# mklawonn/Scene-Graph-GAN

Hardware: AMD Instinct MI355X
Metric: triples/sec (G+D step) (higher is better)
Workload: dtype f32 (conv operands scaled per tensor and split into 2 fp16 pieces, round-to-nearest = 23 significant bits, 3 fp16 MFMAs per product, f32 accumulate; native-f32 figure and parity in the same line); 1 GPU; BASELINE.json configs[1] (1xMI355X, batch 64, 224x224, vocab 1000): batch 64 per GPU, 224x224 synthetic images, vocab 1000, 3-token triples, 1 critic update + 1 generator update per step (WGAN-GP lambda=10, TF-Adam); global_batch=64, critic_iters=1, parallelism=dp1, conv_precision_mode=2, schedule=two-stream; per-kernel figures from serial steps

## Files before the change

### scene-graph-gan_amd/build.py

```python
from __future__ import annotations

import hashlib
import os
import subprocess
import sys
from concurrent.futures import ThreadPoolExecutor

HERE = os.path.dirname(os.path.abspath(__file__))
CSRC = os.path.join(HERE, "csrc")
OUT_DIR = os.path.join(HERE, "_build")
LIB_PATH = os.path.join(HERE, "libsgg_hip.so")
ARCH = "gfx950"
HIPCC = os.environ.get("HIPCC", "/opt/rocm/bin/hipcc")
NO_PACKED_FP32 = ["-Xclang", "-target-feature", "-Xclang", "-packed-fp32-ops"]
FLAGS = ["-O3", "-std=c++17", "-fPIC", "--offload-arch=" + ARCH, "-fno-gpu-rdc", "-Wall", "-Wno-unused-function",
         "-ffp-contract=fast"] + NO_PACKED_FP32


def sources():
    return sorted(os.path.join(CSRC, f) for f in os.listdir(CSRC) if f.endswith(".hip"))


def _digest(paths):
    h = hashlib.sha256()
    for p in sorted(paths):
        with open(p, "rb") as f:
            h.update(p.encode())
            h.update(f.read())
    h.update(" ".join(FLAGS).encode())
    return h.hexdigest()


def _compile(src):
    obj = os.path.join(OUT_DIR, os.path.basename(src) + ".o")
    cmd = [HIPCC] + FLAGS + ["-I", CSRC, "-c", src, "-o", obj]
    r = subprocess.run(cmd, capture_output=True, text=True)
    if r.returncode != 0:
        raise RuntimeError("hipcc failed for %s:\n%s\n%s" % (src, r.stdout, r.stderr))
    err = "\n".join(l for l in r.stderr.splitlines() if "is not a recognized feature for this target" not in l)
    return obj, err


OBJDUMP = os.environ.get("LLVM_OBJDUMP", os.path.join(os.path.dirname(os.path.dirname(os.path.realpath(HIPCC))), "lib", "llvm", "bin",
                                                      "llvm-objdump"))


M0_ASM_KERNELS = ("conv_wgrad_dma", "conv_s2_kernel")


def check_device_code(lib_path: str = LIB_PATH) -> int:
    import re
    import shutil
    tmp = os.path.join(OUT_DIR, "disasm")
    shutil.rmtree(tmp, ignore_errors=True)
    os.makedirs(tmp)
    copy = os.path.join(tmp, "lib.so")
    shutil.copy(lib_path, copy)
    if not os.path.exists(OBJDUMP):
# ... 54 lines not shown
    srcs = sources()
    headers = [os.path.join(CSRC, f) for f in os.listdir(CSRC) if f.endswith(".h")]
    stamp = os.path.join(OUT_DIR, "stamp")
    dig = _digest(srcs + headers)
    if not force and os.path.exists(LIB_PATH) and os.path.exists(stamp) and open(stamp).read() == dig:
        return LIB_PATH
    with ThreadPoolExecutor(max_workers=min(6, len(srcs))) as ex:
        results = list(ex.map(_compile, srcs))
    if verbose:
        for _, err in results:
            if err.strip():
                print(err, file=sys.stderr)
    objs = [o for o, _ in results]
    cmd = [HIPCC, "-shared", "-fPIC", "--offload-arch=" + ARCH, "-o", LIB_PATH] + objs
    r = subprocess.run(cmd, capture_output=True, text=True)
    if r.returncode != 0:
        raise RuntimeError("link failed:\n%s\n%s" % (r.stdout, r.stderr))
    check_device_code(LIB_PATH)
    with open(stamp, "w") as f:
        f.write(dig)
    return LIB_PATH


if __name__ == "__main__":
    print(build(force="--force" in sys.argv, verbose=True))
```

### scene-graph-gan_amd/csrc/conv_gather.hip

```cpp
#include "split16.h"
#include "mma_f32.h"
#include "conv_halo.h"
#include <stdlib.h>

struct GatherClass {
  int Hm, Wm, M;
  int nth, ntw;
  int oy, ox;
  int kh0, kw0, kstep;
  int ooy, oox;
  int mtiles;
};

struct GatherParams {
  const float* src;
  const float* wm;
  const float* bias;
  float* out;
  const void* w_split;
  const float* amax_src;
  const float* amax_w;
  int B, Hs, Ws, C;
  int N;
  int Ho, Wo;
// ... 800 lines not shown
    h.src_s16 = operand_format & 1;
    h.cu_cap = cu_cap;
    SGG_CHECK_ARG((size_t)B * Hi * Wi * Cin * sizeof(float) < 0x80000000ull, "sgg_conv2d_nhwc_fwd: input exceeds 2 GiB");
    sgg_halo_launch(h, precision, st);
    SGG_LAUNCH_CHECK("sgg_conv2d_nhwc_fwd(halo)");
    return SGG_OK;
  }
  if (w_split_layout == 3) {
    SGG_CHECK_ARG(w_split && sgg_s2d_applicable(KH, KW, stride, Hi, Wi, Cin, Cout, precision) && pad_t == 1 && pad_l == 1,
                  "sgg_conv2d_nhwc_fwd: w_split_layout 3 needs 5x5 stride 2, 32 -> 32 channels, H %% 16 == W %% 16 == 0, precision 2 or 3 "
                  "(sgg_conv_wsplit_layout)");
    SGG_CHECK_ARG((size_t)B * Hi * Wi * Cin * sizeof(float) < 0x80000000ull, "sgg_conv2d_nhwc_fwd: input exceeds 2 GiB");
    HaloParams h;
    h.src = x; h.wfrag = w_split; h.bias = bias; h.out = y; h.amax_src = amax_x; h.amax_w = amax_w; h.tile_stats = tile_stats;
    h.ln_stats = ln_stats; h.ln_gamma = ln_gamma; h.ln_beta = ln_beta;
    h.B = B; h.H = Ho; h.W = Wo; h.C = 4 * Cin; h.N = Cout; h.bh = Ho / 8; h.bw = Wo / 8; h.nblk = B * h.bh * h.bw; h.flip = 0;
    h.src_bytes = (unsigned)((size_t)B * Hi * Wi * Cin * sizeof(float));
    h.w_bytes = (unsigned)((size_t)9 * 4 * Cin * Cout * sizeof(float));
    sgg_halo_dense_strides(h);
    h.in_rs = 2 * Wi * Cin; h.in_ps = 2 * Cin; h.in_cA = Wi * Cin; h.in_cB = Cin;
    h.ln_nc = Cin;
    h.src_s16 = operand_format & 1;
    h.cu_cap = cu_cap;
    sgg_halo_launch(h, precision, st);
    SGG_LAUNCH_CHECK("sgg_conv2d_nhwc_fwd(s2d)");
    return SGG_OK;
  }
  if (w_split_layout == 2) {
    SGG_CHECK_ARG(w_split && sgg_s2_applicable(KH, KW, stride, B, Hi, Wi, Cin, Cout, precision) && pad_t == 1 && pad_l == 1,
                  "sgg_conv2d_nhwc_fwd: w_split_layout 2 needs 5x5 stride 2 on an even grid, Cout %% 128 == 0, precision 2 or 3 "
                  "(sgg_conv_wsplit_layout)");
    SGG_CHECK_ARG((size_t)B * Hi * Wi * Cin * sizeof(float) < 0x80000000ull && (size_t)B * Ho * Wo * Cout * sizeof(float) < 0x80000000ull,
                  "sgg_conv2d_nhwc_fwd: tensor exceeds 2 GiB");
    SGG_CHECK_ARG(!tile_stats || sgg_s2_stats_per_sample(Ho, Wo, Cout) > 0, "sgg_conv2d_nhwc_fwd: tile_stats need Ho*Wo %% 224 == 0 here");
    S2Params q;
    q.src = x; q.wfrag = w_split; q.bias = bias; q.out = y; q.amax_src = amax_x; q.amax_w = amax_w; q.tile_stats = tile_stats;
    q.ln_stats = ln_stats; q.ln_gamma = ln_gamma; q.ln_beta = ln_beta;
    q.B = B; q.Ho = Ho; q.Wo = Wo; q.C = Cin; q.N = Cout; q.M = B * Ho * Wo; q.nbands = sgg_cdiv(q.M, 224); q.pitch = Wo;
    q.src_bytes = (unsigned)((size_t)B * Hi * Wi * Cin * sizeof(float));
    q.w_bytes = (unsigned)((size_t)25 * Cin * Cout * sizeof(float));
    q.src_s16 = operand_format & 1;
    q.cu_cap = cu_cap;
    sgg_s2_launch(q, 0, precision, st);
    SGG_LAUNCH_CHECK("sgg_conv2d_nhwc_fwd(s2)");
    return SGG_OK;
  }
// ... 46 lines not shown
    h.src_bytes = (unsigned)((size_t)B * Ho * Wo * Cout * sizeof(float));
    h.w_bytes = (unsigned)((size_t)9 * Cin * Cout * sizeof(float));
    sgg_halo_dense_strides(h);
    h.frag16 = w_split_layout == 4;
    h.src_s16 = operand_format & 1;
    sgg_halo_launch(h, precision, (hipStream_t)stream);
    SGG_LAUNCH_CHECK("sgg_conv2d_nhwc_dgrad(halo)");
    return SGG_OK;
  }
  if (w_split_layout == 3) {
    SGG_CHECK_ARG(w_split && sgg_s2d_applicable(KH, KW, stride, Hi, Wi, Cin, Cout, precision) && pad_t == 1 && pad_l == 1 &&
                      Hi == 2 * Ho && Wi == 2 * Wo,
                  "sgg_conv2d_nhwc_dgrad: w_split_layout 3 needs 5x5 stride 2, 32 -> 32 channels, H %% 16 == W %% 16 == 0, precision 2 or 3 "
                  "(sgg_conv_wsplit_layout)");
    HaloParams h;
    h.src = dy; h.wfrag = w_split; h.bias = nullptr; h.out = dx; h.amax_src = amax_dy; h.amax_w = amax_w; h.tile_stats = nullptr;
    h.ln_stats = nullptr; h.ln_gamma = nullptr; h.ln_beta = nullptr;
    h.B = B; h.H = Ho; h.W = Wo; h.C = Cout; h.N = 4 * Cin; h.bh = Ho / 8; h.bw = Wo / 8; h.nblk = B * h.bh * h.bw; h.flip = 1;
    h.src_bytes = (unsigned)((size_t)B * Ho * Wo * Cout * sizeof(float));
    h.w_bytes = (unsigned)((size_t)9 * 4 * Cin * Cout * sizeof(float));
    sgg_halo_dense_strides(h);
    h.out_rs = 2 * Wi * Cin; h.out_ps = 2 * Cin; h.out_nA = Wi * Cin; h.out_nB = Cin;
    h.src_s16 = operand_format & 1;
    sgg_halo_launch(h, precision, (hipStream_t)stream);
    SGG_LAUNCH_CHECK("sgg_conv2d_nhwc_dgrad(s2d)");
    return SGG_OK;
  }
  if (w_split_layout == 2) {
    SGG_CHECK_ARG(w_split && sgg_s2_applicable(KH, KW, stride, B, Hi, Wi, Cout, Cin, precision) && pad_t == 1 && pad_l == 1 &&
                      Hi == 2 * Ho && Wi == 2 * Wo,
                  "sgg_conv2d_nhwc_dgrad: w_split_layout 2 needs 5x5 stride 2 on an even grid, Cin %% 128 == 0, precision 2 or 3 "
                  "(sgg_conv_wsplit_layout)");
    SGG_CHECK_ARG((size_t)B * Hi * Wi * Cin * sizeof(float) < 0x80000000ull && (size_t)B * Ho * Wo * Cout * sizeof(float) < 0x80000000ull,
                  "sgg_conv2d_nhwc_dgrad: tensor exceeds 2 GiB");
    S2Params q;
    q.src = dy; q.wfrag = w_split; q.bias = nullptr; q.out = dx; q.amax_src = amax_dy; q.amax_w = amax_w; q.tile_stats = nullptr;
    q.ln_stats = nullptr; q.ln_gamma = nullptr; q.ln_beta = nullptr;
    q.B = B; q.Ho = Ho; q.Wo = Wo; q.C = Cout; q.N = Cin; q.M = B * Ho * Wo; q.nbands = sgg_cdiv(q.M, 224); q.pitch = Wo;
    q.src_bytes = (unsigned)((size_t)B * Ho * Wo * Cout * sizeof(float));
    q.w_bytes = (unsigned)((size_t)25 * Cin * Cout * sizeof(float));
    q.src_s16 = operand_format & 1;
    q.cu_cap = 0;
    sgg_s2_launch(q, 1, precision, (hipStream_t)stream);
    SGG_LAUNCH_CHECK("sgg_conv2d_nhwc_dgrad(s2)");
    return SGG_OK;
  }
// ... 27 lines not shown
```

### scene-graph-gan_amd/csrc/conv_halo.h

```cpp
#pragma once
#include "sgg_common.h"

struct HaloParams {
  const float* src;
  const void* wfrag;
  const float* bias;
  float* out;
  const float* amax_src;
  const float* amax_w;
  float* tile_stats;
  const float* ln_stats;
  const float* ln_gamma;
  const float* ln_beta;
  int B, H, W, C, N;
  int bh, bw, nblk;
  int flip;
  unsigned src_bytes, w_bytes;
  int gx;
  int in_rs, in_ps, in_cA, in_cB;
  int out_rs, out_ps, out_nA, out_nB;
  int ln_nc;
  int frag16;
  int src_s16;
  int cu_cap;
};
inline int sgg_persist_cus(int cu_cap) { return (cu_cap > 0 && cu_cap < SGG_PERSIST_CUS_PER_XCD) ? cu_cap : SGG_PERSIST_CUS_PER_XCD; }
inline void sgg_halo_dense_strides(HaloParams& h) {
  h.in_rs = h.W * h.C; h.in_ps = h.C; h.in_cA = 64; h.in_cB = 32;
  h.out_rs = h.W * h.N; h.out_ps = h.N; h.out_nA = 64; h.out_nB = 32;
  h.ln_nc = h.C;
  h.frag16 = 0;
  h.src_s16 = 0;
  h.cu_cap = 0;
}

int sgg_halo_applicable(int KH, int KW, int stride, int H, int W, int C, int N, int precision);
int sgg_s2d_applicable(int KH, int KW, int stride, int Hi, int Wi, int Cin, int Cout, int precision);
int sgg_halo_stats_cols(int N);
void sgg_halo_launch(const HaloParams& p, int precision, hipStream_t st);
int sgg_halo_pc_applicable(int C, int N, int precision);
int sgg_halo_pc64_applicable(int C, int N, int precision);
void sgg_halo_pc_launch(const HaloParams& p, int precision, hipStream_t st);

struct WgradHaloPlan {
  int ct, nt;
  int nbs;
  int spw;
  int pairs, pairs_n;
  int nsplit;
  int stages;
  int nslabs;
  int geo;
  int R, pc, xslots;
  size_t ws_bytes;
};
int sgg_wgrad_halo_plan(int B, int H, int W, int Cin, int Cout, int KH, int KW, int stride, WgradHaloPlan* pl);
// ... 43 lines not shown
```

### scene-graph-gan_amd/csrc/conv_halo.hip

```cpp
#include "split16.h"
#include "conv_halo.h"
#include <type_traits>
#include <stdlib.h>

constexpr int SGG_HALO_DB_MAX = 65536;
#define HALO_PITCH 12
#define HALO_BLKB (10 * HALO_PITCH * 64)

__device__ __forceinline__ int halo_sw(int ry, int rx) { return ((rx >> 2) & 1) | ((ry & 1) << 1); }

template <int NB, int BN, int WGM, int WGN, bool HALF, bool PREFETCH, bool ONECH, bool LNP, bool ONE = false, int WB = 1>
__global__ __launch_bounds__(64 * WGM * WGN, 2) void conv_halo3_kernel(HaloParams p) {
  static_assert(PREFETCH && WB == 1, "patch prefetch, one block per wave");
  constexpr int P = ONE ? 1 : 2;
  constexpr int WN = BN / WGN, TM = 2 * WB, TN = WN / 32;
  constexpr int THREADS = 64 * WGM * WGN;
  static_assert((WGM * WGN == 4 || WGM * WGN == 2) && NB * 64 / WGM == 64 * WB && WN % 32 == 0 && TN >= 1,
                "a wave owns WB 8x8 blocks x WN columns");
  constexpr int PLANEB = NB * HALO_BLKB;
  constexpr int ITEMS = NB * 400;
  constexpr int NPASS = (ITEMS + THREADS - 1) / THREADS;
  constexpr bool DB = (2 * P * PLANEB <= SGG_HALO_DB_MAX) && THREADS == 256;
  __shared__ __attribute__((aligned(16))) unsigned char lds[(DB ? 2 : 1) * P * PLANEB];
  __shared__ __attribute__((aligned(16))) float lnp_s[LNP ? 1024 : 4];

  const int ntiles_n = p.N / BN;
  const int mtiles = (p.nblk + NB - 1) / NB;
  const int xcd = blockIdx.x & 7, jx = blockIdx.x >> 3;
  const int nt = jx % ntiles_n;
  const int tstride = p.gx / ntiles_n;
  const int mt_begin = (int)(((long long)xcd * mtiles) >> 3) + jx / ntiles_n;
  const int mt_end = (int)(((long long)(xcd + 1) * mtiles) >> 3);
  if (mt_begin >= mt_end) return;
  const int n0 = nt * BN;
  const int tid = threadIdx.x, lane = tid & 63;
  const int wave = __builtin_amdgcn_readfirstlane(tid >> 6);
// ... 27 lines not shown
      lnp_s[512 + c] = p.ln_beta[c];
    }
    __syncthreads();
  }
  float ld_mu[NB], ld_rs[NB];
  int ld_cc = 0, ld_bad = 0;

  int s_grow[NB], s_by[NB], s_bx[NB];
#pragma unroll
  for (int j = 0; j < NB; ++j) {
    const int beta = mt_begin * NB + j;
    s_grow[j] = beta / p.bw;
    s_bx[j] = beta % p.bw;
    s_by[j] = s_grow[j] % p.bh;
  }
  int s_tile = mt_begin, s_cc = 0;
  const int nch = p.C >> 5;
  const int adv_rows = (tstride * NB) / p.bw, adv_cols = (tstride * NB) % p.bw;

  f32x4 pre[NPASS][2];
  auto stage_load = [&]() __attribute__((always_inline)) {
    unsigned base[NB];
    int bbits[NB];
#pragma unroll
    for (int j = 0; j < NB; ++j) {
      const bool dead = (s_tile >= mt_end) | (s_tile * NB + j >= p.nblk);
      base[j] = (unsigned)(((s_grow[j] * 8 - 1) * p.in_rs + (s_bx[j] * 8 - 1) * p.in_ps + (s_cc >> 1) * p.in_cA + (s_cc & 1) * p.in_cB) * 4);
      bbits[j] = dead ? 15 : ((s_by[j] == 0) | ((s_by[j] == p.bh - 1) << 1) | ((s_bx[j] == 0) << 2) | ((s_bx[j] == p.bw - 1) << 3));
      if (dead) base[j] = SGG_OOB;
    }
    if constexpr (LNP) {
      ld_cc = s_cc;
      ld_bad = 0;
#pragma unroll
      for (int j = 0; j < NB; ++j) {
        int b = s_grow[j] / p.bh;
        b = b < p.B ? b : p.B - 1;
        ld_mu[j] = p.ln_stats[2 * b];
        ld_rs[j] = p.ln_stats[2 * b + 1];
      }
    }
#pragma unroll
    for (int j = 0; j < NPASS; ++j) {
      const int blk = (it_meta[j] >> 24) & 3;
      unsigned b0 = base[0];
      int bb = bbits[0];
#pragma unroll
      for (int k = 1; k < NB; ++k) {
        b0 = blk == k ? base[k] : b0;
        bb = blk == k ? bbits[k] : bb;
// ... 29 lines not shown
        const int blk = (it_meta[j] >> 24) & 3;
        float mu = ld_mu[0], rs = ld_rs[0];
#pragma unroll
        for (int k = 1; k < NB; ++k) {
          mu = blk == k ? ld_mu[k] : mu;
          rs = blk == k ? ld_rs[k] : rs;
        }
        const int cb = ((ld_cc * 32) & (p.ln_nc - 1)) + ((it_meta[j] >> 26) & 3) * 8;
        ln_elu8(pre[j][0], pre[j][1], lnp_s + cb, lnp_s + 512 + cb, mu, rs, (ld_bad >> j) & 1);
      }
      u32x4 pl[P];
      if constexpr (LNP || !HALF) split8<P, HALF>(pre[j][0], pre[j][1], sa, pl);
      else stage_planes<P, HALF>(pre[j][0], pre[j][1], sa, p.src_s16, pl);
      if ((it_meta[j] >> 28) & 1) {
#pragma unroll
        for (int pp = 0; pp < P; ++pp) *reinterpret_cast<u32x4*>(dst + pp * PLANEB + (it_meta[j] & 0xfffff)) = pl[pp];
      }
    }
  };

  const unsigned w_lane = (unsigned)((n0 + wn0) >> 5) * 4096u + (unsigned)lane * 16u;
  const unsigned w_slab = (unsigned)(p.N >> 5) * 4096u;
  u32x4 rb[2][TN][2][P];
  auto load_b = [&](auto par_c, int cc, int tap) {
    constexpr int par = decltype(par_c)::value;
    const unsigned base = (unsigned)(tap * nch + cc) * w_slab + w_lane;
#pragma unroll
    for (int tn = 0; tn < TN; ++tn)
#pragma unroll
      for (int ks = 0; ks < 2; ++ks)
#pragma unroll
        for (int pp = 0; pp < P; ++pp)
          rb[par][tn][ks][pp] = __builtin_bit_cast(u32x4, buf_load4(rs_w, base + (unsigned)(tn * 4096 + ks * 2048 + pp * 1024)));
  };

  f32x16 acc[TM][TN];
  acc_zero<TM, TN>(acc);

  const int i = lane & 31, h = lane >> 5;
  const int pyl = i >> 3, pxl = i & 7;
  int cur = 0;

  u32x4 a[2][TM][2][P];
  auto read_a_ks = [&](auto buf_c, int tap, auto ks0_c, auto nks_c) {
    constexpr int buf = decltype(buf_c)::value, ks0 = decltype(ks0_c)::value, nks = decltype(nks_c)::value;
    const int kh = tap / 3, kw = tap % 3;
    const int dyy = p.flip ? 2 - kh : kh, dxx = p.flip ? 2 - kw : kw;
    int pyv = pyl, pxv = pxl;
    asm volatile("" : "+v"(pyv), "+v"(pxv));
    const unsigned char* patch_w = lds + (DB ? cur * (P * PLANEB) : 0) + wblk * HALO_BLKB;
#pragma unroll
    for (int tm = 0; tm < TM; ++tm) {
      const int ry = (tm & 1) * 4 + pyv + dyy, rx = pxv + dxx;
      const unsigned char* row = patch_w + (tm >> 1) * HALO_BLKB + (ry * HALO_PITCH + rx) * 64;
      const int hs = halo_sw(ry, rx);
#pragma unroll
      for (int ks = ks0; ks < ks0 + nks; ++ks)
#pragma unroll
        for (int pp = 0; pp < P; ++pp)
          a[buf][tm][ks][pp] = *reinterpret_cast<const u32x4*>(row + pp * PLANEB + (((2 * ks + h) ^ hs) << 4));
    }
  };
  auto read_a = [&](auto buf_c, int tap) { read_a_ks(buf_c, tap, std::integral_constant<int, 0>{}, std::integral_constant<int, 2>{}); };
  auto mma_kstep = [&](auto par_c, auto ks_c) {
    constexpr int par = decltype(par_c)::value, ks = decltype(ks_c)::value;
#pragma unroll
    for (int tm = 0; tm < TM; ++tm)
#pragma unroll
      for (int tn = 0; tn < TN; ++tn) {
        f32x16 d = acc[tm][tn];
        if constexpr (P == 2) {
          d = mfma16<HALF>(a[par][tm][ks][1], rb[par][tn][ks][0], d);
          d = mfma16<HALF>(a[par][tm][ks][0], rb[par][tn][ks][1], d);
        }
        d = mfma16<HALF>(a[par][tm][ks][0], rb[par][tn][ks][0], d);
        acc[tm][tn] = d;
      }
  };
  auto tap_body = [&](auto par_c, auto tap_c, int cc) {
    constexpr int par = decltype(par_c)::value, tap = decltype(tap_c)::value;
    const int ncc = (cc + 1 == nch) ? 0 : cc + 1;
    load_b(std::integral_constant<int, par ^ 1>{}, tap == 8 ? ncc : cc, tap == 8 ? 0 : tap + 1);
    if constexpr (tap == 6) stage_load();
    __builtin_amdgcn_sched_barrier(0);
    if constexpr (DB && tap == 8) stage_write(lds + (cur ^ 1) * (P * PLANEB));
    SGG_PRIO_HI();
    mma_kstep(par_c, std::integral_constant<int, 0>{});
    __builtin_amdgcn_sched_barrier(0);
    if constexpr (tap < 8) read_a(std::integral_constant<int, par ^ 1>{}, tap + 1);
    __builtin_amdgcn_sched_barrier(0);
    mma_kstep(par_c, std::integral_constant<int, 1>{});
    SGG_PRIO_LO();
    __builtin_amdgcn_sched_barrier(0);
  };
  auto chunk = [&](auto par0_c, int cc) {
    constexpr int par0 = decltype(par0_c)::value;
    read_a(par0_c, 0);
#define SGG_TAP(T) tap_body(std::integral_constant<int, (par0 + T) & 1>{}, std::integral_constant<int, T>{}, cc)
    SGG_TAP(0); SGG_TAP(1); SGG_TAP(2); SGG_TAP(3); SGG_TAP(4); SGG_TAP(5); SGG_TAP(6); SGG_TAP(7); SGG_TAP(8);
#undef SGG_TAP
    if constexpr (DB) {
      cur ^= 1;
      asm volatile("s_waitcnt lgkmcnt(0)" ::: "memory");
      __builtin_amdgcn_s_barrier();
    } else {
      asm volatile("s_waitcnt lgkmcnt(0)" ::: "memory");
      __builtin_amdgcn_s_barrier();
      stage_write(lds);
      asm volatile("s_waitcnt lgkmcnt(0)" ::: "memory");
      __builtin_amdgcn_s_barrier();
    }
  };

  int o_grow[WB], o_bx[WB];
#pragma unroll
  for (int wb = 0; wb < WB; ++wb) {
    const int beta = mt_begin * NB + wblk + wb;
    o_grow[wb] = beta / p.bw;
    o_bx[wb] = beta % p.bw;
  }
  const unsigned o_lane_b = (unsigned)(((4 * h + (lane & 3)) * p.out_ps) + ((lane & 31) >> 2) * 4) * 4u;
  int o_goff[TN];
#pragma unroll
  for (int tn = 0; tn < TN; ++tn) {
    const int gi = ((n0 + wn0) >> 5) + tn;
    o_goff[tn] = (gi >> 1) * p.out_nA + (gi & 1) * p.out_nB;
  }
  const float us_a = ldexpf(1.f, -ea), us_b = ldexpf(1.f, -eb);
  float bias_v[TN];
#pragma unroll
  for (int tn = 0; tn < TN; ++tn) bias_v[tn] = p.bias ? p.bias[n0 + wn0 + tn * 32 + acc_col(lane)] : 0.f;
  const int wn = p.out_rs;

  stage_load();
  load_b(std::integral_constant<int, 0>{}, 0, 0);
  stage_write(lds);
  asm volatile("s_waitcnt lgkmcnt(0)" ::: "memory");
  __builtin_amdgcn_s_barrier();

  auto epilogue = [&](int tile) {
#pragma unroll
    for (int wb = 0; wb < WB; ++wb) {
      const int beta = tile * NB + wblk + wb;
      const bool live = beta < p.nblk;
      const char* ob = reinterpret_cast<const char*>(p.out + (size_t)(o_grow[wb] * 8) * wn + (size_t)(o_bx[wb] * 8) * p.out_ps);
      float lsum = 0.f;
#pragma unroll
      for (int tn = 0; tn < TN; ++tn)
#pragma unroll
        for (int t2 = 0; t2 < 2; ++t2)
#pragma unroll
          for (int r = 0; r < 16; ++r) {
            const int tm = 2 * wb + t2;
            const float v = HALF ? fmaf(acc[tm][tn][r] * us_a, us_b, bias_v[tn]) : acc[tm][tn][r] + bias_v[tn];
            acc[tm][tn][r] = v;
            lsum += v;
          }
      if (live) {
#pragma unroll
        for (int tn = 0; tn < TN; ++tn)
#pragma unroll
// ... 17 lines not shown
#pragma unroll
            for (int r = 0; r < 16; ++r) {
              const float d = acc[2 * wb + t2][tn][r] - mean_w;
              q += d * d;
              dm = fmaxf(dm, fabsf(d));
            }
        q = wave_sum(q);
        dm = wave_max(dm);
        if (lane == 0 && live) {
          float* o = p.tile_stats + ((size_t)beta * (p.N / WN) + (n0 + wn0) / WN) * SGG_TS;
          o[0] = (float)(64 * WN);
          o[1] = mean_w;
          o[2] = q;
          o[3] = dm;
        }
      }
      o_bx[wb] += adv_cols;
      o_grow[wb] += adv_rows;
      if (o_bx[wb] >= p.bw) { o_bx[wb] -= p.bw; ++o_grow[wb]; }
    }
    acc_zero<TM, TN>(acc);
  };

  if constexpr (ONECH) {
    for (int tile = mt_begin; tile < mt_end; tile += 2 * tstride) {
      chunk(std::integral_constant<int, 0>{}, 0);
      epilogue(tile);
      if (tile + tstride < mt_end) {
        chunk(std::integral_constant<int, 1>{}, 0);
        epilogue(tile + tstride);
      }
    }
  } else {
    for (int tile = mt_begin; tile < mt_end; tile += tstride) {
      for (int cc = 0; cc < nch; cc += 2) {
        chunk(std::integral_constant<int, 0>{}, cc);
        chunk(std::integral_constant<int, 1>{}, cc + 1);
      }
      epilogue(tile);
    }
  }
}

template <bool HALF>
__global__ void split_weights_frag_kernel(const float* __restrict__ in, u32x4* __restrict__ out, int taps, int N, int C,
                                          const float* __restrict__ amax) {
  const long long idx = (long long)blockIdx.x * blockDim.x + threadIdx.x;
  const int nch = C >> 5, ntl = N >> 5;
  if (idx >= (long long)taps * nch * ntl * 128) return;
  const int lane = (int)(idx & 63), ks = (int)((idx >> 6) & 1);
  long long r = idx >> 7;
  const int ntile = (int)(r % ntl); r /= ntl;
  const int cc = (int)(r % nch);
  const int tap = (int)(r / nch);
  const int n = ntile * 32 + (lane & 31), k = cc * 32 + ks * 16 + 8 * (lane >> 5);
  const float* src = in + ((size_t)tap * N + n) * C + k;
  const float scale = HALF ? ldexpf(1.f, scale_exp_from_amax(*amax)) : 1.f;
  u32x4 pl[2];
  split8<2, HALF>(*reinterpret_cast<const f32x4*>(src), *reinterpret_cast<const f32x4*>(src + 4), scale, pl);
  const size_t o = ((((size_t)(tap * nch + cc) * ntl + ntile) * 2 + ks) * 2) * 64 + lane;
  out[o] = pl[0];
  out[o + 64] = pl[1];
}

// ... 16 lines not shown
  SGG_LAUNCH_CHECK("sgg_conv_s2d_weights");
  return SGG_OK;
}

int sgg_s2d_applicable(int KH, int KW, int stride, int Hi, int Wi, int Cin, int Cout, int precision) {
  return KH == 5 && KW == 5 && stride == 2 && Hi > 0 && Wi > 0 && Hi % 16 == 0 && Wi % 16 == 0 && Cin == 32 && Cout == 32 &&
         sgg_prec_resident(precision);
}

int sgg_halo_applicable(int KH, int KW, int stride, int H, int W, int C, int N, int precision) {
  return KH == 3 && KW == 3 && stride == 1 && H > 0 && W > 0 && H % 8 == 0 && W % 8 == 0 && (C == 32 || C % 64 == 0) && N % 32 == 0 &&
         sgg_prec_resident(precision);
}

int sgg_halo_stats_cols(int N) { return N % 128 == 0 ? 64 : 32; }

void sgg_halo_launch(const HaloParams& p_, int precision, hipStream_t st) {
  if (p_.frag16) {
    sgg_halo_pc_launch(p_, precision, st);
    return;
  }
  HaloParams p = p_;
  const bool half = sgg_prec_half(precision), one = sgg_prec_one(precision);
#define SGG_HALO(NB, BN, WGM, WGN)                                                                           \
  do {                                                                                                       \
    const int mtiles = sgg_cdiv(p.nblk, NB), ntn = p.N / BN;                                                 \
    int per_xcd = sgg_cdiv(mtiles, 8) * ntn;                           \
    const int cap = sgg_persist_cus(p.cu_cap) * 8 / (WGM * WGN);      \
    int gx = per_xcd < cap ? per_xcd : cap;                                                                  \
    gx = sgg_cdiv(gx, ntn) * ntn;                                                                            \
    p.gx = gx;                                                                                               \
    const dim3 grid((unsigned)(8 * gx));                                                                     \
    const dim3 blk(64 * WGM * WGN);                                                                          \
    if (one) {                                                                                                                          \
      if (half && p.C == 32) hipLaunchKernelGGL((conv_halo3_kernel<NB, BN, WGM, WGN, true, true, true, false, true, 1>), grid, blk, 0, st, p);   \
      else if (half) hipLaunchKernelGGL((conv_halo3_kernel<NB, BN, WGM, WGN, true, true, false, false, true, 1>), grid, blk, 0, st, p);      \
      else if (p.C == 32) hipLaunchKernelGGL((conv_halo3_kernel<NB, BN, WGM, WGN, false, true, true, false, true, 1>), grid, blk, 0, st, p); \
      else hipLaunchKernelGGL((conv_halo3_kernel<NB, BN, WGM, WGN, false, true, false, false, true, 1>), grid, blk, 0, st, p);               \
    } else if (p.ln_stats) {                                                                                                            \
      if (half && p.C == 32) hipLaunchKernelGGL((conv_halo3_kernel<NB, BN, WGM, WGN, true, true, true, true, false, 1>), grid, blk, 0, st, p);   \
      else if (half) hipLaunchKernelGGL((conv_halo3_kernel<NB, BN, WGM, WGN, true, true, false, true, false, 1>), grid, blk, 0, st, p);      \
      else if (p.C == 32) hipLaunchKernelGGL((conv_halo3_kernel<NB, BN, WGM, WGN, false, true, true, true, false, 1>), grid, blk, 0, st, p); \
      else hipLaunchKernelGGL((conv_halo3_kernel<NB, BN, WGM, WGN, false, true, false, true, false, 1>), grid, blk, 0, st, p);               \
    } else if (half && p.C == 32) hipLaunchKernelGGL((conv_halo3_kernel<NB, BN, WGM, WGN, true, true, true, false, false, 1>), grid, blk, 0, st, p); \
    else if (half) hipLaunchKernelGGL((conv_halo3_kernel<NB, BN, WGM, WGN, true, true, false, false, false, 1>), grid, blk, 0, st, p);       \
    else if (p.C == 32) hipLaunchKernelGGL((conv_halo3_kernel<NB, BN, WGM, WGN, false, true, true, false, false, 1>), grid, blk, 0, st, p);  \
    else hipLaunchKernelGGL((conv_halo3_kernel<NB, BN, WGM, WGN, false, true, false, false, false, 1>), grid, blk, 0, st, p);                \
// ... 68 lines not shown
```

### scene-graph-gan_amd/lib.py

```python
from __future__ import annotations

import ctypes
import os
from ctypes import c_char_p, c_float, c_int, c_longlong, c_size_t, c_void_p

import torch

_HERE = os.path.dirname(os.path.abspath(__file__))
LIB_PATH = os.path.join(_HERE, "libsgg_hip.so")

_vp, _i, _f, _sz, _ll = c_void_p, c_int, c_float, c_size_t, c_longlong

SIGNATURES = {
    "sgg_version": (_i, []),
    "sgg_last_error": (c_char_p, []),
    "sgg_device_info": (_i, [_vp, _vp, _vp, _vp, _i]),
    "sgg_hwio_to_hwoi": (_i, [_vp, _vp, _i, _i, _i, _vp]),
    "sgg_conv_split_weights": (_i, [_vp, _vp, _ll, _i, _vp, _vp]),
    "sgg_absmax": (_i, [_vp, _ll, _vp, _vp]),
    "sgg_conv_wsplit_layout": (_i, [_i] * 8),
    "sgg_conv_wsplit_layout_presplit": (_i, [_i] * 8),
    "sgg_conv_s2d_weights": (_i, [_vp, _vp, _i, _i, _vp]),
    "sgg_conv_prepare_weights": (_i, [_vp, _i, _i, _vp]),
    "sgg_conv_split_weights_frag": (_i, [_vp, _vp, _i, _i, _i, _i, _vp, _vp]),
# ... 279 lines not shown
        for d, lay in zip(arr, layers):
            w = lay["w"]
            kh, kw, ci, co = w.shape
            self._dev(w, lay["w_fwd"], lay.get("w3"), lay.get("w3_fwd"), lay.get("ws_fwd"), lay.get("ws_bwd"), lay.get("amax"))
            d.w, d.w_hwoi = _p(w), _p(lay["w_fwd"])
            d.w3, d.w3_hwoi = _p(lay.get("w3")), _p(lay.get("w3_fwd"))
            d.ws_fwd, d.ws_bwd, d.amax = _p(lay.get("ws_fwd")), _p(lay.get("ws_bwd")), _p(lay.get("amax"))
            d.taps, d.cin, d.cout, d.layout_fwd, d.layout_bwd = kh * kw, ci, co, lay["ws_layout"], lay["ws_layout_bwd"]
        return arr

    def prepare_weights(self, descs):
        self._check(self.lib.sgg_conv_prepare_weights(ctypes.addressof(descs), len(descs), self.conv_precision, self._stream()),
                    "sgg_conv_prepare_weights")

    def conv_tile_stats_count(self, y_shape, cin, k=0, stride=0, layout=0):
        return self.lib.sgg_conv2d_nhwc_fwd_tile_stats(y_shape[1], y_shape[2], cin, y_shape[3], k, k, stride, self.conv_precision,
                                                       layout)

    def halo_pc_symbol(self, lnp=False, presplit=False, n_out=128):
        dma = presplit and not lnp and self.conv_precision == 2
        return "conv_halo3_pc_kernel<%s,%s,%s,%d>" % ("true" if self.conv_precision == 2 else "false", "true" if lnp else "false",
                                                      "true" if dma else "false", 2 if n_out % 128 == 0 else 4)

    def halo_symbol(self, n_out, n_in, lnp=False):
        tile = "2,128,2,2" if n_out % 128 == 0 else ("2,64,2,2" if n_out % 64 == 0 else "2,32,2,1")
        return "conv_halo3_kernel<%s,%s,%s,%s,%s,%s,1>" % (tile, "true" if self.conv_precision in (1, 2) else "false", "true",
                                                           "true" if n_in == 32 else "false", "true" if lnp else "false",
                                                           "true" if self.conv_precision in (1, 4) else "false")

    def s2_symbol(self, dgrad, m_positions=1 << 30, n_out=128, stats=True, lnp=False, presplit=False):
        mt = 7
        dma = presplit and not lnp and self.conv_precision == 2
        return "conv_s2_kernel<%s,%s,%d,%s,%s,%s,%d>" % ("true" if dgrad else "false", "true" if self.conv_precision in (1, 2) else "false", mt,
                                                         "true" if self.conv_precision in (1, 4) else "false", "true" if lnp else "false",
                                                         "true" if dma else "false",
                                                         8 if dma and n_out % 256 == 0 and -(-m_positions // 224) * (n_out // 256) > 128 else 4)

    def conv_fwd(self, x, w_hwio, w_fwd, bias, y, stride, w_split=None, amax_x=None, amax_w=None, tile_stats=None, w_split_layout=0,
                 ln=None, x_s16=False, cu_cap=0):
        self._dev(x, w_fwd, bias, y)
        ln_s, ln_g, ln_b = ln if ln is not None else (None, None, None)
        self._dev(ln_s, ln_g, ln_b)
        d = self._conv_dims(x.shape, w_hwio.shape, stride)
        assert tuple(y.shape) == (d[0], d[4], d[5], d[6]) and x.is_contiguous() and y.is_contiguous()
        flops = 2.0 * d[0] * d[4] * d[5] * d[6] * d[7] * d[8] * d[3]
        sym = "conv_c3_fwd_kernel" if d[3] == 3 else (self.halo_pc_symbol(ln is not None, x_s16, d[6]) if w_split_layout == 4 else
                                                             self.halo_symbol(d[6], d[3], ln is not None) if w_split_layout == 1 else
                                                             self.halo_symbol(d[6], 4 * d[3], ln is not None) if w_split_layout == 3 else
                                                             self.s2_symbol(False, d[0] * d[4] * d[5], d[6], tile_stats is not None, ln is not None, x_s16) if w_split_layout == 2 else
                                                             self.gather_symbol(d[6], w_split is not None))
        nb = 0.0
        if d[3] != 3:
            amax_x, amax_w = self._amax_or_compute(x, amax_x, 0), self._amax_or_compute(w_fwd, amax_w, 1)
        else:
            nb = 4.0 * (x.numel() + y.numel())
        self._check(self._timed(sym, flops, lambda: self.lib.sgg_conv2d_nhwc_fwd(
            _p(x), _p(w_fwd), _p(w_split), _p(bias), _p(y), *d, self.conv_precision, w_split_layout, _p(amax_x), _p(amax_w),
            _p(tile_stats), _p(ln_s), _p(ln_g), _p(ln_b), int(bool(x_s16)) | ((int(cu_cap) & 63) << 8), self._stream()), nb),
            "sgg_conv2d_nhwc_fwd")

    def conv_dgrad(self, dy, w_hwio, dx, stride, w_split=None, amax_dy=None, amax_w=None, w_split_layout=0, dy_s16=False):
        self._dev(dy, w_hwio, dx)
        d = self._conv_dims(dx.shape, w_hwio.shape, stride)
        assert tuple(dy.shape) == (d[0], d[4], d[5], d[6]) and dy.is_contiguous() and dx.is_contiguous()
        flops = 2.0 * d[0] * d[4] * d[5] * d[6] * d[7] * d[8] * d[3]
        amax_dy, amax_w = self._amax_or_compute(dy, amax_dy, 0), self._amax_or_compute(w_hwio, amax_w, 1)
        sym = self.halo_pc_symbol(False, dy_s16, d[3]) if w_split_layout == 4 else self.halo_symbol(d[3], d[6]) if w_split_layout == 1 else (self.halo_symbol(4 * d[3], d[6]) if w_split_layout == 3 else
                                                                          self.s2_symbol(True, d[0] * d[4] * d[5], d[3], False, False, dy_s16) if w_split_layout == 2 else
                                                                          self.gather_symbol(d[3], w_split is not None))
        self._check(self._timed(sym, flops, lambda: self.lib.sgg_conv2d_nhwc_dgrad(
            _p(dy), _p(w_hwio), _p(w_split), _p(dx), *d, self.conv_precision, w_split_layout, _p(amax_dy), _p(amax_w),
# ... 366 lines not shown
```

Measured before the change: 1527 triples/sec.

## Skip structurally zero taps in space-to-depth 5x5 stride-2 halo convolution

Adds a dedicated space-to-depth variant of the halo conv kernel. It iterates over the four channel classes with compile-time tap masks, so the 3x3 virtual taps that correspond to zero-padded weights of the 5x5 kernel are skipped. Only 25 of the 36 tap-class pairs issue MFMAs and weight loads, and the pipeline staging points are recomputed per run. The cost is more template code and a persistent grid fixed at 2 waves. The dgrad path also sets the s2d flag, but the flip case still falls back to the old kernel.

```diff
diff --git a/scene-graph-gan_amd/build.py b/scene-graph-gan_amd/build.py
--- a/scene-graph-gan_amd/build.py
+++ b/scene-graph-gan_amd/build.py
@@ -21,19 +21,19 @@
     return sorted(os.path.join(CSRC, f) for f in os.listdir(CSRC) if f.endswith(".hip"))
 
 
-def _digest(paths):
+def _digest(paths, flags=()):
     h = hashlib.sha256()
     for p in sorted(paths):
         with open(p, "rb") as f:
             h.update(p.encode())
             h.update(f.read())
-    h.update(" ".join(FLAGS).encode())
+    h.update(" ".join(FLAGS + list(flags)).encode())
     return h.hexdigest()
 
 
-def _compile(src):
-    obj = os.path.join(OUT_DIR, os.path.basename(src) + ".o")
-    cmd = [HIPCC] + FLAGS + ["-I", CSRC, "-c", src, "-o", obj]
+def _compile(src, out_dir=OUT_DIR, flags=()):
+    obj = os.path.join(out_dir, os.path.basename(src) + ".o")
+    cmd = [HIPCC] + FLAGS + list(flags) + ["-I", CSRC, "-c", src, "-o", obj]
     r = subprocess.run(cmd, capture_output=True, text=True)
     if r.returncode != 0:
         raise RuntimeError("hipcc failed for %s:\n%s\n%s" % (src, r.stdout, r.stderr))
@@ -134,5 +134,23 @@
     return LIB_PATH
 
 
+def build_variant(name: str, flags, force: bool = False) -> str:
+    out_dir = os.path.join(OUT_DIR, name)
+    os.makedirs(out_dir, exist_ok=True)
+    lib_path, stamp = os.path.join(out_dir, "libsgg_hip.so"), os.path.join(out_dir, "stamp")
+    srcs = sources()
+    dig = _digest(srcs + [os.path.join(CSRC, f) for f in os.listdir(CSRC) if f.endswith(".h")], flags)
+    if not force and os.path.exists(lib_path) and os.path.exists(stamp) and open(stamp).read() == dig:
+        return lib_path
+    with ThreadPoolExecutor(max_workers=min(6, len(srcs))) as ex:
+        objs = [o for o, _ in ex.map(lambda src: _compile(src, out_dir, flags), srcs)]
+    r = subprocess.run([HIPCC, "-shared", "-fPIC", "--offload-arch=" + ARCH, "-o", lib_path] + objs, capture_output=True, text=True)
+    if r.returncode != 0:
+        raise RuntimeError("link failed:\n%s\n%s" % (r.stdout, r.stderr))
+    with open(stamp, "w") as f:
+        f.write(dig)
+    return lib_path
+
+
 if __name__ == "__main__":
     print(build(force="--force" in sys.argv, verbose=True))
diff --git a/scene-graph-gan_amd/csrc/conv_gather.hip b/scene-graph-gan_amd/csrc/conv_gather.hip
--- a/scene-graph-gan_amd/csrc/conv_gather.hip
+++ b/scene-graph-gan_amd/csrc/conv_gather.hip
@@ -846,6 +846,7 @@
     h.ln_nc = Cin;
     h.src_s16 = operand_format & 1;
     h.cu_cap = cu_cap;
+    h.s2d = 1;
     sgg_halo_launch(h, precision, st);
     SGG_LAUNCH_CHECK("sgg_conv2d_nhwc_fwd(s2d)");
     return SGG_OK;
@@ -938,6 +939,7 @@
     sgg_halo_dense_strides(h);
     h.out_rs = 2 * Wi * Cin; h.out_ps = 2 * Cin; h.out_nA = Wi * Cin; h.out_nB = Cin;
     h.src_s16 = operand_format & 1;
+    h.s2d = 1;
     sgg_halo_launch(h, precision, (hipStream_t)stream);
     SGG_LAUNCH_CHECK("sgg_conv2d_nhwc_dgrad(s2d)");
     return SGG_OK;
diff --git a/scene-graph-gan_amd/csrc/conv_halo.h b/scene-graph-gan_amd/csrc/conv_halo.h
--- a/scene-graph-gan_amd/csrc/conv_halo.h
+++ b/scene-graph-gan_amd/csrc/conv_halo.h
@@ -23,6 +23,7 @@
   int frag16;
   int src_s16;
   int cu_cap;
+  int s2d;
 };
 inline int sgg_persist_cus(int cu_cap) { return (cu_cap > 0 && cu_cap < SGG_PERSIST_CUS_PER_XCD) ? cu_cap : SGG_PERSIST_CUS_PER_XCD; }
 inline void sgg_halo_dense_strides(HaloParams& h) {
@@ -32,6 +33,7 @@
   h.frag16 = 0;
   h.src_s16 = 0;
   h.cu_cap = 0;
+  h.s2d = 0;
 }
 
 int sgg_halo_applicable(int KH, int KW, int stride, int H, int W, int C, int N, int precision);
diff --git a/scene-graph-gan_amd/csrc/conv_halo.hip b/scene-graph-gan_amd/csrc/conv_halo.hip
--- a/scene-graph-gan_amd/csrc/conv_halo.hip
+++ b/scene-graph-gan_amd/csrc/conv_halo.hip
@@ -9,9 +9,45 @@
 
 __device__ __forceinline__ int halo_sw(int ry, int rx) { return ((rx >> 2) & 1) | ((ry & 1) << 1); }
 
-template <int NB, int BN, int WGM, int WGN, bool HALF, bool PREFETCH, bool ONECH, bool LNP, bool ONE = false, int WB = 1>
-__global__ __launch_bounds__(64 * WGM * WGN, 2) void conv_halo3_kernel(HaloParams p) {
+constexpr bool s2d_live(int tap, int q) { return !((tap / 3 == 0 && (q >> 1) == 0) || (tap % 3 == 0 && (q & 1) == 0)); }
+constexpr int s2d_fwd_cls(int k) { return k & 3; }
+constexpr unsigned halo_run_all(int TN) {
+  unsigned m = 0;
+  for (int tap = 0; tap < 9; ++tap) m |= ((1u << TN) - 1u) << (2 * tap);
+  return m;
+}
+constexpr unsigned s2d_run_fwd(int q) {
+  unsigned m = 0;
+  for (int tap = 0; tap < 9; ++tap) m |= (unsigned)s2d_live(tap, q) << (2 * tap);
+  return m;
+}
+constexpr int run_tiles(unsigned m, int tap) { return tap < 9 ? (int)((m >> (2 * tap)) & 3u) : 0; }
+constexpr int run_next(unsigned m, int tap) {
+  for (int t = tap + 1; t < 9; ++t)
+    if (run_tiles(m, t)) return t;
+  return 9;
+}
+constexpr int run_first(unsigned m) { return run_next(m, -1); }
+constexpr int run_before(unsigned m, int tap) {
+  int n = 0;
+  for (int t = 0; t < tap; ++t) n += run_tiles(m, t) != 0;
+  return n;
+}
+constexpr int run_count(unsigned m) { return run_before(m, 9); }
+constexpr int run_stage_tap(unsigned m) {
+  int t = run_first(m);
+  for (int k = 0; k < run_count(m) - 3; ++k) t = run_next(m, t);
+  return t;
+}
+template <unsigned M> struct HaloRun {
+  static constexpr unsigned masks = M;
+  static_assert(run_count(M) >= 3, "a run stages the next patch at its third-from-last tap");
+};
+
+template <int NB, int BN, int WGM, int WGN, bool HALF, bool PREFETCH, bool ONECH, bool LNP, bool ONE, int WB, bool S2D>
+__device__ __forceinline__ void conv_halo3_body(const HaloParams& p) {
   static_assert(PREFETCH && WB == 1, "patch prefetch, one block per wave");
+  static_assert(!S2D || (!ONECH && BN == 32 && WGN == 1), "space-to-depth view, forward: 128 virtual channels x 32 columns");
   constexpr int P = ONE ? 1 : 2;
   constexpr int WN = BN / WGN, TM = 2 * WB, TN = WN / 32;
   constexpr int THREADS = 64 * WGM * WGN;
@@ -85,10 +121,11 @@
   auto stage_load = [&]() __attribute__((always_inline)) {
     unsigned base[NB];
     int bbits[NB];
+    const int scc = S2D ? s2d_fwd_cls(s_cc) : s_cc;
 #pragma unroll
     for (int j = 0; j < NB; ++j) {
       const bool dead = (s_tile >= mt_end) | (s_tile * NB + j >= p.nblk);
-      base[j] = (unsigned)(((s_grow[j] * 8 - 1) * p.in_rs + (s_bx[j] * 8 - 1) * p.in_ps + (s_cc >> 1) * p.in_cA + (s_cc & 1) * p.in_cB) * 4);
+      base[j] = (unsigned)(((s_grow[j] * 8 - 1) * p.in_rs + (s_bx[j] * 8 - 1) * p.in_ps + (scc >> 1) * p.in_cA + (scc & 1) * p.in_cB) * 4);
       bbits[j] = dead ? 15 : ((s_by[j] == 0) | ((s_by[j] == p.bh - 1) << 1) | ((s_bx[j] == 0) << 2) | ((s_bx[j] == p.bw - 1) << 3));
       if (dead) base[j] = SGG_OOB;
     }
@@ -164,16 +201,19 @@
   const unsigned w_lane = (unsigned)((n0 + wn0) >> 5) * 4096u + (unsigned)lane * 16u;
   const unsigned w_slab = (unsigned)(p.N >> 5) * 4096u;
   u32x4 rb[2][TN][2][P];
-  auto load_b = [&](auto par_c, int cc, int tap) {
-    constexpr int par = decltype(par_c)::value;
+  auto load_b = [&](auto par_c, auto run_c, auto tap_c, int cc) {
+    constexpr int par = decltype(par_c)::value, tap = decltype(tap_c)::value;
+    using R = decltype(run_c);
     const unsigned base = (unsigned)(tap * nch + cc) * w_slab + w_lane;
 #pragma unroll
-    for (int tn = 0; tn < TN; ++tn)
+    for (int tn = 0; tn < TN; ++tn) {
+      if (!((run_tiles(R::masks, tap) >> tn) & 1)) continue;
 #pragma unroll
       for (int ks = 0; ks < 2; ++ks)
 #pragma unroll
         for (int pp = 0; pp < P; ++pp)
           rb[par][tn][ks][pp] = __builtin_bit_cast(u32x4, buf_load4(rs_w, base + (unsigned)(tn * 4096 + ks * 2048 + pp * 1024)));
+    }
   };
 
   f32x16 acc[TM][TN];
@@ -204,12 +244,13 @@
     }
   };
   auto read_a = [&](auto buf_c, int tap) { read_a_ks(buf_c, tap, std::integral_constant<int, 0>{}, std::integral_constant<int, 2>{}); };
-  auto mma_kstep = [&](auto par_c, auto ks_c) {
-    constexpr int par = decltype(par_c)::value, ks = decltype(ks_c)::value;
+  auto mma_kstep = [&](auto par_c, auto ks_c, auto tiles_c) {
+    constexpr int par = decltype(par_c)::value, ks = decltype(ks_c)::value, tiles = decltype(tiles_c)::value;
 #pragma unroll
     for (int tm = 0; tm < TM; ++tm)
 #pragma unroll
       for (int tn = 0; tn < TN; ++tn) {
+        if (!((tiles >> tn) & 1)) continue;
         f32x16 d = acc[tm][tn];
         if constexpr (P == 2) {
           d = mfma16<HALF>(a[par][tm][ks][1], rb[par][tn][ks][0], d);
@@ -219,26 +260,33 @@
         acc[tm][tn] = d;
       }
   };
-  auto tap_body = [&](auto par_c, auto tap_c, int cc) {
+  auto tap_body = [&](auto par_c, auto tap_c, auto run_c, auto nrun_c, int cc, int ncc) {
     constexpr int par = decltype(par_c)::value, tap = decltype(tap_c)::value;
-    const int ncc = (cc + 1 == nch) ? 0 : cc + 1;
-    load_b(std::integral_constant<int, par ^ 1>{}, tap == 8 ? ncc : cc, tap == 8 ? 0 : tap + 1);
-    if constexpr (tap == 6) stage_load();
+    constexpr unsigned M = decltype(run_c)::masks, MN = decltype(nrun_c)::masks;
+    constexpr int nxt = run_next(M, tap);
+    constexpr bool last = nxt == 9;
+    if constexpr (last) load_b(std::integral_constant<int, par ^ 1>{}, nrun_c, std::integral_constant<int, run_first(MN)>{}, ncc);
+    else load_b(std::integral_constant<int, par ^ 1>{}, run_c, std::integral_constant<int, nxt>{}, cc);
+    if constexpr (tap == run_stage_tap(M)) stage_load();
     __builtin_amdgcn_sched_barrier(0);
-    if constexpr (DB && tap == 8) stage_write(lds + (cur ^ 1) * (P * PLANEB));
+    if constexpr (DB && last) stage_write(lds + (cur ^ 1) * (P * PLANEB));
     SGG_PRIO_HI();
-    mma_kstep(par_c, std::integral_constant<int, 0>{});
+    mma_kstep(par_c, std::integral_constant<int, 0>{}, std::integral_constant<int, run_tiles(M, tap)>{});
     __builtin_amdgcn_sched_barrier(0);
-    if constexpr (tap < 8) read_a(std::integral_constant<int, par ^ 1>{}, tap + 1);
+    if constexpr (!last) read_a(std::integral_constant<int, par ^ 1>{}, nxt);
     __builtin_amdgcn_sched_barrier(0);
-    mma_kstep(par_c, std::integral_constant<int, 1>{});
+    mma_kstep(par_c, std::integral_constant<int, 1>{}, std::integral_constant<int, run_tiles(M, tap)>{});
     SGG_PRIO_LO();
     __builtin_amdgcn_sched_barrier(0);
   };
-  auto chunk = [&](auto par0_c, int cc) {
+  auto chunk = [&](auto par0_c, auto run_c, auto nrun_c, int cc, int ncc) {
     constexpr int par0 = decltype(par0_c)::value;
-    read_a(par0_c, 0);
-#define SGG_TAP(T) tap_body(std::integral_constant<int, (par0 + T) & 1>{}, std::integral_constant<int, T>{}, cc)
+    constexpr unsigned M = decltype(run_c)::masks;
+    if constexpr (S2D) asm volatile("" : "+s"(cc), "+s"(ncc));
+    read_a(par0_c, run_first(M));
+#define SGG_TAP(T)                                                                                                              \
+  if constexpr (run_tiles(M, T) != 0)                                                                                           \
+    tap_body(std::integral_constant<int, (par0 + run_before(M, T)) & 1>{}, std::integral_constant<int, T>{}, run_c, nrun_c, cc, ncc)
     SGG_TAP(0); SGG_TAP(1); SGG_TAP(2); SGG_TAP(3); SGG_TAP(4); SGG_TAP(5); SGG_TAP(6); SGG_TAP(7); SGG_TAP(8);
 #undef SGG_TAP
     if constexpr (DB) {
@@ -274,11 +322,13 @@
   for (int tn = 0; tn < TN; ++tn) bias_v[tn] = p.bias ? p.bias[n0 + wn0 + tn * 32 + acc_col(lane)] : 0.f;
   const int wn = p.out_rs;
 
+  auto prologue = [&](auto run_c, int cc) {
+    load_b(std::integral_constant<int, 0>{}, run_c, std::integral_constant<int, run_first(decltype(run_c)::masks)>{}, cc);
+    stage_write(lds);
+    asm volatile("s_waitcnt lgkmcnt(0)" ::: "memory");
+    __builtin_amdgcn_s_barrier();
+  };
   stage_load();
-  load_b(std::integral_constant<int, 0>{}, 0, 0);
-  stage_write(lds);
-  asm volatile("s_waitcnt lgkmcnt(0)" ::: "memory");
-  __builtin_amdgcn_s_barrier();
 
   auto epilogue = [&](int tile) {
 #pragma unroll
@@ -342,24 +392,76 @@
     acc_zero<TM, TN>(acc);
   };
 
-  if constexpr (ONECH) {
+  using IC0 = std::integral_constant<int, 0>;
+  using IC1 = std::integral_constant<int, 1>;
+  auto tiles_onech = [&](auto run_c) {
+    constexpr int odd = run_count(decltype(run_c)::masks) & 1;
+    prologue(run_c, 0);
+    if constexpr (odd) {
+      for (int tile = mt_begin; tile < mt_end; tile += 2 * tstride) {
+        chunk(IC0{}, run_c, run_c, 0, 0);
+        epilogue(tile);
+        if (tile + tstride < mt_end) {
+          chunk(IC1{}, run_c, run_c, 0, 0);
+          epilogue(tile + tstride);
+        }
+      }
+    } else {
+      for (int tile = mt_begin; tile < mt_end; tile += tstride) {
+        chunk(IC0{}, run_c, run_c, 0, 0);
+        epilogue(tile);
+      }
+    }
+  };
+  if constexpr (!S2D) {
+    using RunAll = HaloRun<halo_run_all(TN)>;
+    if constexpr (ONECH) {
+      tiles_onech(RunAll{});
+    } else {
+      prologue(RunAll{}, 0);
+      for (int tile = mt_begin; tile < mt_end; tile += tstride) {
+        for (int cc = 0; cc < nch; cc += 2) {
+          chunk(IC0{}, RunAll{}, RunAll{}, cc, cc + 1);
+          chunk(IC1{}, RunAll{}, RunAll{}, cc + 1, cc + 2 == nch ? 0 : cc + 2);
+        }
+        epilogue(tile);
+      }
+    }
+  } else {
+    constexpr int c0 = s2d_fwd_cls(0), c1 = s2d_fwd_cls(1), c2 = s2d_fwd_cls(2), c3 = s2d_fwd_cls(3);
+    using R0 = HaloRun<s2d_run_fwd(c0)>;
+    using R1 = HaloRun<s2d_run_fwd(c1)>;
+    using R2 = HaloRun<s2d_run_fwd(c2)>;
+    using R3 = HaloRun<s2d_run_fwd(c3)>;
+    static_assert(((1 << c0) | (1 << c1) | (1 << c2) | (1 << c3)) == 15, "each class once per tile");
+    auto tile4 = [&](auto par0_c) {
+      constexpr int q0 = decltype(par0_c)::value;
+      constexpr int q1 = q0 + run_count(R0::masks), q2 = q1 + run_count(R1::masks), q3 = q2 + run_count(R2::masks);
+      chunk(std::integral_constant<int, q0 & 1>{}, R0{}, R1{}, c0, c1);
+      chunk(std::integral_constant<int, q1 & 1>{}, R1{}, R2{}, c1, c2);
+      chunk(std::integral_constant<int, q2 & 1>{}, R2{}, R3{}, c2, c3);
+      chunk(std::integral_constant<int, q3 & 1>{}, R3{}, R0{}, c3, c0);
+    };
+    static_assert((run_count(R0::masks) + run_count(R1::masks) + run_count(R2::masks) + run_count(R3::masks)) == 25, "5 x 5 taps");
+    prologue(R0{}, c0);
     for (int tile = mt_begin; tile < mt_end; tile += 2 * tstride) {
-      chunk(std::integral_constant<int, 0>{}, 0);
+      tile4(IC0{});
       epilogue(tile);
       if (tile + tstride < mt_end) {
-        chunk(std::integral_constant<int, 1>{}, 0);
+        tile4(IC1{});
         epilogue(tile + tstride);
       }
     }
-  } else {
-    for (int tile = mt_begin; tile < mt_end; tile += tstride) {
-      for (int cc = 0; cc < nch; cc += 2) {
-        chunk(std::integral_constant<int, 0>{}, cc);
-        chunk(std::integral_constant<int, 1>{}, cc + 1);
-      }
-      epilogue(tile);
-    }
-  }
+  }
+}
+
+template <int NB, int BN, int WGM, int WGN, bool HALF, bool PREFETCH, bool ONECH, bool LNP, bool ONE = false, int WB = 1>
+__global__ __launch_bounds__(64 * WGM * WGN, 2) void conv_halo3_kernel(HaloParams p) {
+  conv_halo3_body<NB, BN, WGM, WGN, HALF, PREFETCH, ONECH, LNP, ONE, WB, false>(p);
+}
+template <int NB, int BN, int WGM, int WGN, bool HALF, bool PREFETCH, bool ONECH, bool LNP, bool ONE = false, int WB = 1>
+__global__ __launch_bounds__(64 * WGM * WGN, 2) void conv_halo3_s2d_kernel(HaloParams p) {
+  conv_halo3_body<NB, BN, WGM, WGN, HALF, PREFETCH, ONECH, LNP, ONE, WB, true>(p);
 }
 
 template <bool HALF>
@@ -422,7 +524,26 @@
   }
   HaloParams p = p_;
   const bool half = sgg_prec_half(precision), one = sgg_prec_one(precision);
-#define SGG_HALO(NB, BN, WGM, WGN)                                                                           \
+  auto persistent_grid = [&](int NB, int BN, int waves) {
+    const int mtiles = sgg_cdiv(p.nblk, NB), ntn = p.N / BN;
+    const int per_xcd = sgg_cdiv(mtiles, 8) * ntn;
+    const int cap = sgg_persist_cus(p.cu_cap) * 8 / waves;
+    p.gx = sgg_cdiv(per_xcd < cap ? per_xcd : cap, ntn) * ntn;
+    return dim3((unsigned)(8 * p.gx));
+  };
+#ifndef SGG_S2D_FULL_SLOTS
+  if (p.s2d && !p.flip) {
+    const dim3 grid = persistent_grid(2, 32, 2);
+#define SGG_S2D(H, L, O) hipLaunchKernelGGL((conv_halo3_s2d_kernel<2, 32, 2, 1, H, true, false, L, O, 1>), grid, dim3(128), 0, st, p)
+    if (one) { if (half) SGG_S2D(true, false, true); else SGG_S2D(false, false, true); }
+    else if (p.ln_stats) { if (half) SGG_S2D(true, true, false); else SGG_S2D(false, true, false); }
+    else if (half) SGG_S2D(true, false, false);
+    else SGG_S2D(false, false, false);
+#undef SGG_S2D
+    return;
+  }
+#endif
+#define SGG_HALO(NB, BN, WGM, WGN)                                                                        \
   do {                                                                                                       \
     const int mtiles = sgg_cdiv(p.nblk, NB), ntn = p.N / BN;                                                 \
     int per_xcd = sgg_cdiv(mtiles, 8) * ntn;                           \
diff --git a/scene-graph-gan_amd/lib.py b/scene-graph-gan_amd/lib.py
--- a/scene-graph-gan_amd/lib.py
+++ b/scene-graph-gan_amd/lib.py
@@ -325,9 +325,9 @@
         return "conv_halo3_pc_kernel<%s,%s,%s,%d>" % ("true" if self.conv_precision == 2 else "false", "true" if lnp else "false",
                                                       "true" if dma else "false", 2 if n_out % 128 == 0 else 4)
 
-    def halo_symbol(self, n_out, n_in, lnp=False):
+    def halo_symbol(self, n_out, n_in, lnp=False, s2d=False):
         tile = "2,128,2,2" if n_out % 128 == 0 else ("2,64,2,2" if n_out % 64 == 0 else "2,32,2,1")
-        return "conv_halo3_kernel<%s,%s,%s,%s,%s,%s,1>" % (tile, "true" if self.conv_precision in (1, 2) else "false", "true",
+        return "conv_halo3%s_kernel<%s,%s,%s,%s,%s,%s,1>" % ("_s2d" if s2d else "", tile, "true" if self.conv_precision in (1, 2) else "false", "true",
                                                            "true" if n_in == 32 else "false", "true" if lnp else "false",
                                                            "true" if self.conv_precision in (1, 4) else "false")
 
@@ -349,7 +349,7 @@
         flops = 2.0 * d[0] * d[4] * d[5] * d[6] * d[7] * d[8] * d[3]
         sym = "conv_c3_fwd_kernel" if d[3] == 3 else (self.halo_pc_symbol(ln is not None, x_s16, d[6]) if w_split_layout == 4 else
                                                              self.halo_symbol(d[6], d[3], ln is not None) if w_split_layout == 1 else
-                                                             self.halo_symbol(d[6], 4 * d[3], ln is not None) if w_split_layout == 3 else
+                                                             self.halo_symbol(d[6], 4 * d[3], ln is not None, s2d=True) if w_split_layout == 3 else
                                                              self.s2_symbol(False, d[0] * d[4] * d[5], d[6], tile_stats is not None, ln is not None, x_s16) if w_split_layout == 2 else
                                                              self.gather_symbol(d[6], w_split is not None))
         nb = 0.0
```

Result: no change. 1532 triples/sec, median of 6 (+0.3%).
